# imjaegyun/super_resolution

Hardware: AMD Instinct MI355X
Metric: SR output megapixels/sec, HAT-S x4, 1280x720 LR in (higher is better)
Workload: dtype bf16; 1 GPU; HAT-S x4, one 3x720x1280 LR frame per GPU, full-frame forward; upscale=4, parallelism=dp1

## Files before the change

super_resolution_amd/build.py:

```python
from __future__ import annotations

import os
import subprocess
import sys
from concurrent.futures import ThreadPoolExecutor

HERE = os.path.dirname(os.path.abspath(__file__))
CSRC = os.path.join(HERE, "csrc")
LIB = os.path.join(HERE, "libhat_mi355x.so")
SOURCES = ["hat_conv.hip", "hat_conv64r.hip", "hat_attn.hip", "hat_misc.hip", "hat_ffn.hip", "hat_ffn2.hip", "hat_tail3.hip", "hat_tail3l.hip", "hat_pw.hip", "hat_mlp.hip", "hat_cabsq.hip", "hat_esc13.hip", "hat_plan.cpp"]
HEADERS = [os.path.join(CSRC, "hat_common.h"), os.path.join(os.path.dirname(HERE), "include", "hat_mi355x.h")]
FLAGS = ["-O3", "--offload-arch=gfx950", "-fPIC", "-std=c++17", "-Wall", "-Wno-unused-function"]


def _hipcc() -> str:
    for c in (os.environ.get("HIPCC"), "/opt/rocm/bin/hipcc", "hipcc"):
        if c and (os.path.isabs(c) and os.path.exists(c) or not os.path.isabs(c)):
            return c
    raise RuntimeError("hipcc not found")


def _stale(target: str, deps) -> bool:
    if not os.path.exists(target):
        return True
    t = os.path.getmtime(target)
    return any(os.path.getmtime(d) > t for d in deps)


def build(force: bool = False, verbose: bool = True) -> str:
    hipcc = _hipcc()
    objs, jobs = [], []
    for src in SOURCES:
        s = os.path.join(CSRC, src)
        o = os.path.join(CSRC, os.path.splitext(src)[0] + ".o")
        objs.append(o)
        if force or _stale(o, [s] + HEADERS):
            jobs.append([hipcc, *FLAGS, "-c", s, "-o", o])

    def run(cmd):
        if verbose:
            print(" ".join(cmd), flush=True)
        r = subprocess.run(cmd, capture_output=True, text=True)
        if r.returncode != 0:
            raise RuntimeError(f"hipcc failed:\n{' '.join(cmd)}\n{r.stdout}\n{r.stderr}")
        if verbose and r.stderr.strip():
            print(r.stderr, file=sys.stderr)

    with ThreadPoolExecutor(max_workers=4) as ex:
        list(ex.map(run, jobs))
    if force or jobs or _stale(LIB, objs):
        run([hipcc, "--offload-arch=gfx950", "-shared", "-fPIC", "-o", LIB, *objs])
    return LIB


if __name__ == "__main__":
    print(build(force="--force" in sys.argv))
```

super_resolution_amd/csrc/hat_tail3.hip:

```cpp
#include "hat_common.h"

#ifndef T3_ISSUE_ALL
#define T3_ISSUE_ALL 0
#endif
#ifndef T3_APF
#define T3_APF 1
#endif
#ifndef T3_S0RD
#define T3_S0RD 8
#endif
#ifndef T3_ABL
#define T3_ABL 0
#endif
#ifndef T3_USTORE_IL
#define T3_USTORE_IL 1
#endif
#ifndef T3_DMA_LATE
#define T3_DMA_LATE 0
#endif

namespace {

typedef _Float16 h2 __attribute__((ext_vector_type(2)));
typedef _Float16 h8 __attribute__((ext_vector_type(8)));
// ... 415 lines not shown
            };
            const bool pair16 = d.ldn % 8 == 0 && reinterpret_cast<uintptr_t>(d.n_out) % 16 == 0;
            {
                const f32x4 o0 = lnv(0);
                if (valid) {
                    if (4 * g < d.gap_c) gapv += as_stored<bf16_t>(o0);
                    if (d.n16_out != nullptr)
                        Vec4<bf16_t>::store(reinterpret_cast<bf16_t*>(d.n16_out) + ((size_t)b * H * W + pix) * 16 + 4 * g, o0);
                }
                if (pair16) {
                    store_pair_bf16_if(nout, 0, g, o0, lnv(1), valid);
#pragma unroll
                    for (int nt = 2; nt + 1 < NT; nt += 2) store_pair_bf16_if(nout, nt * 16, g, lnv(nt), lnv(nt + 1), valid);
                    if (valid) Vec4<bf16_t>::store(nout + (NT - 1) * 16 + 4 * g, lnv(NT - 1));
                } else if (valid) {
                    Vec4<bf16_t>::store(nout + 4 * g, o0);
#pragma unroll
                    for (int nt = 1; nt < NT; ++nt) Vec4<bf16_t>::store(nout + nt * 16 + 4 * g, lnv(nt));
                }
            }
        }
    }
    if constexpr (DBG & 64) {
        stamp(7);
        if (lane == 0) {
            const size_t wg = ((size_t)blockIdx.z * gridDim.y + blockIdx.y) * gridDim.x + blockIdx.x;
            for (int i = 0; i < 12; ++i) d.gap_out[(wg * T3_WAVES + wave) * 12 + i] = (float)tph[i];
        }
        return;
    }
    if (do_ln && d.gap_out != nullptr) {
        float* red = reinterpret_cast<float*>(smem + T3_WD_OFF);
#pragma unroll
        for (int r = 0; r < 4; ++r) {
            float s = gapv[r];
            s = row_sum16(s);
            if (c16 == 0) red[wave * 16 + 4 * g + r] = s;
        }
        __syncthreads();
        if (tid < 16) {
            float s = 0.f;
#pragma unroll
            for (int w = 0; w < T3_WAVES; ++w) s += red[w * 16 + tid];
            const size_t tile = (size_t)blockIdx.y * gridDim.x + blockIdx.x;
            d.gap_out[((size_t)b * gridDim.x * gridDim.y + tile) * 16 + tid] = tid < d.gap_c ? s : 0.f;
        }
    }
}

}

#ifndef HAT_TAIL3_NO_ENTRY
int hat_tail3_launch_c180(const HatHabTailDesc& h, void* stream);

extern "C" int hat_hab_tail3(const HatHabTailDesc* dp, void* stream) {
    if (!dp) return HAT_EINVAL;
    const HatHabTailDesc& h = *dp;
    const HatFfnDesc& d = h.ffn;
    if (!d.t_in || !d.t_out || d.t_in == d.t_out || !d.w1f || !d.dww || !d.w2f || !d.b2) return HAT_EINVAL;
    if (d.B < 1 || d.H < 1 || d.W < 1 || d.chunks < 1 || d.m_in) return HAT_EINVAL;
    if (d.dtype != HAT_BF16) return HAT_EUNSUPPORTED;
    if (d.C == 180) return (d.chunks == 12 && h.reserved1 == 0) ? hat_tail3_launch_c180(h, stream) : HAT_EINVAL;
    if (d.C != T3_C) return HAT_EUNSUPPORTED;
    if (d.ln1_g && (!d.ln1_b || !d.n_out || d.ldn < d.C || d.ldn % 4 || d.gap_c < 0 || d.gap_c > 16 || d.gap_c % 4)) return HAT_EINVAL;
    if (!h.n || !h.y16 || !h.c1 || !h.w_aggr || !h.wf || !h.bias_b || h.ldn_in < T3_C || h.ldn_in % 8) return HAT_EINVAL;
    const T3Aggr ag{reinterpret_cast<const bf16_t*>(h.n), reinterpret_cast<const bf16_t*>(h.y16), reinterpret_cast<const bf16_t*>(h.c1),
                    reinterpret_cast<const char*>(h.w_aggr), reinterpret_cast<const char*>(h.wf), h.bias_b, h.ldn_in};
    const int th = h.reserved1 & 3;
    if ((h.reserved1 & ~3) != 0) return HAT_EINVAL;
    if ((th & 1) && reinterpret_cast<uintptr_t>(d.t_in) % 8) return HAT_EINVAL;
    if ((th & 2) && reinterpret_cast<uintptr_t>(d.t_out) % 16) return HAT_EINVAL;
    void (*kern)(const HatFfnDesc, const T3Aggr) = th == 0 ? tail3_kernel<0, 0> : th == 1 ? tail3_kernel<0, 1> : th == 2 ? tail3_kernel<0, 2> : tail3_kernel<0, 3>;
    hipError_t e = hipFuncSetAttribute(reinterpret_cast<const void*>(kern), hipFuncAttributeMaxDynamicSharedMemorySize, T3_LDS);
    if (e != hipSuccess) return (int)e;
    dim3 grid((d.W + 15) / 16, (d.H + T3_ROWS - 1) / T3_ROWS, d.B);
    HAT_LAUNCH(kern, grid, dim3(256), T3_LDS, reinterpret_cast<hipStream_t>(stream), d, ag);
    return hat_check_launch();
}
#endif
```

super_resolution_amd/engine.py:

```python
from __future__ import annotations

import collections
import dataclasses
import math
import os
import threading
from typing import Dict, Optional

import torch

from . import ops
from .ops import (ACT_GELU, ACT_LRELU, ACT_NONE, O_NCHW_F32, O_NHWC_F32, O_NHWC_T, O_PIXSHUF_T, X_NCHW_F32_MEAN, X_NHWC_F32, X_NHWC_T)

RGB_MEAN = (0.4488, 0.4371, 0.4040)


def _r8(x: int) -> int:
    return (x + 7) // 8 * 8


def _r4(x: int) -> int:
    return (x + 3) // 4 * 4


@dataclasses.dataclass(frozen=True)
class Options:
    no_n16: bool = False
    no_t16: bool = False
    emu_t16: Optional[torch.dtype] = None
    no_fused_ffn: bool = False
    ffn_v1: bool = False
    no_hab_tail: bool = False
    tail_v2: bool = False
    no_cab_fold: bool = False
    no_cab_sweep: bool = False
    no_esc13: bool = False
    esc_side: bool = False
    one_stream: bool = False
    no_attn_log2: bool = False
    no_ocab_mlp: bool = False
    no_ocab_qkv: bool = False
    no_bf16_conv_in: bool = False
    no_conv_ln: bool = False

    @classmethod
    def from_env(cls, env=None) -> "Options":
        env = os.environ if env is None else env
        get = lambda name: env.get("HAT_" + name.upper(), "")
        any_value = ("no_cab_fold", "no_cab_sweep", "no_ocab_mlp", "no_ocab_qkv", "no_bf16_conv_in", "no_conv_ln")
        kw = {k.name: (get(k.name) != "" if k.name in any_value else get(k.name) == "1") for k in dataclasses.fields(cls)}
        return cls(**dict(kw, emu_t16={"fp16": torch.float16, "bf16": torch.bfloat16}.get(get("emu_t16"))))


class _ESC:

    def __init__(self, sd, core: str, plk_key: str, pdim: int, ksize: int, C: int, dtype: int, dev):
        f32 = dict(dtype=torch.float32, device=dev)
        self.pdim, self.ksize = pdim, ksize
        self.w1 = sd[core + ".plk.dwc_proj.1.weight"].detach().reshape(pdim // 2, pdim).to(**f32).contiguous()
        self.b1 = sd[core + ".plk.dwc_proj.1.bias"].detach().to(**f32).contiguous()
        self.w2 = sd[core + ".plk.dwc_proj.3.weight"].detach().reshape(pdim * 9, pdim // 2).to(**f32).contiguous()
        self.b2 = sd[core + ".plk.dwc_proj.3.bias"].detach().to(**f32).contiguous()
        lk = ops.pack_conv_weight(sd[plk_key], None, ops.HAT_F32, dev, nt=1)
        kc = ops.KC[dtype] * 3
        self.kpad = -(-(ksize * ksize * _r8(pdim)) // kc) * kc
        self.npad = 16 if pdim <= 16 else 32
        plk = torch.zeros(self.npad, self.kpad, **f32)
        plk[:lk.w.shape[0], :min(self.kpad, lk.kpad)] = lk.w[:self.npad, :min(self.kpad, lk.kpad)]
        self.plk = plk.contiguous()
        self.zero_bias = torch.zeros(self.npad, **f32)
        self.aggr = None
        self.aggr_keys = (core + ".aggr.weight", core + ".aggr.bias")
        self.conv13 = False


class _Packed:

    def __getitem__(self, key):
        try:
            return getattr(self, key)
        except AttributeError:
            raise KeyError(key) from None


class _Hab(_Packed):
    fold = ffn = ffn3 = fc1 = fc2 = bias256 = None
# ... 513 lines not shown
            self._esc_conv(esc, w, w["n"], B, H, W, n16=n16)
        s0.wait_stream(s1)

    def _fold_band(self, f: _Fwd, hb: _Hab, gst):
        w, bd, W, fo = f.w, f.band, f.W, hb.fold
        self._squeeze_chain(f, hb)
        st, c1, lo, own = w["cstat_l"], w["c1"], bd.lo, bd.own
        f.pooled(c1, 8, 8, st, 0)
        f.pooled(c1, 8, 8, st, 24, c0=0, c1=1)
        f.pooled(c1, 8, 8, st, 32, c0=W - 1, c1=W)
        if bd.r0 == 0:
            f.pooled(c1, 8, 8, st, 8, r0=lo, r1=lo + 1)
            f.pooled(c1, 8, 8, st, 40, r0=lo, r1=lo + 1, c0=0, c1=1)
            f.pooled(c1, 8, 8, st, 48, r0=lo, r1=lo + 1, c0=W - 1, c1=W)
        if bd.r1 == bd.Hfull:
            f.pooled(c1, 8, 8, st, 16, r0=lo + own - 1, r1=lo + own)
            f.pooled(c1, 8, 8, st, 56, r0=lo + own - 1, r1=lo + own, c0=0, c1=1)
            f.pooled(c1, 8, 8, st, 64, r0=lo + own - 1, r1=lo + own, c0=W - 1, c1=W)
        yield ("reduce", [(gst[0], gst[1], hb.esc.pdim), (st, w["cstat_g"], 72)])
        ops.cab_fold(None, None, 1, hb.cab0.npad, fo["w2"], fo["b2"], hb.eca_w, hb.eca_w.numel(), fo["ba"],
                     float(self.cfg["conv_scale"]), w["scale"], w["wf"], w["bias_b"], None, B=f.B, H=bd.Hfull, W=W, C_=self.C,
                     mid=hb.cab0.nout, dtype=f.dt, stats=w["cstat_g"], w2f=fo["w2f"])

    def _prologue_plain(self, f: _Fwd, hb: _Hab, gst):
        w, esc, bd, B, H, W, C, ldc = f.w, hb.esc, f.band, f.B, f.H, f.W, self.C, f.ldc
        mid = hb.cab0.nout
        c3 = ops.conv3x3_small if hb.cab0.frag else ops.conv
        c3(hb.cab0, w["n"], w["c1"], **f.geo, ldx=ldc, ldo=_r8(mid), act=ACT_GELU, n_store=_r4(mid))
        c3 = ops.conv3x3_small if hb.cab2.frag else ops.conv
        c3(hb.cab2, w["c1"], w["c2"], **f.geo, ldx=_r8(mid), ldo=ldc, colsum=w["colsum"])
        if bd is None:
            ops.eca_scale(w["colsum"], w["tiles"], hb.cab2.npad, f.N, hb.eca_w, hb.eca_w.numel(),
                          float(self.cfg["conv_scale"]), w["eca_tmp"], w["scale"], B=B, C_=C)
            self._esc_lk(esc, w, w["n"], B, H, W, f.nblk)
            return
        npd = hb.cab2.npad
        el, eg = (w[k].view(-1)[:B * npd].view(B, npd) for k in ("estat_l", "estat_g"))
        f.pooled(w["c2"], ldc, C, el)
        yield ("reduce", [(gst[0], gst[1], esc.pdim), (el, eg, _r4(C))])
        ops.eca_scale(eg, 1, npd, bd.Hfull * W, hb.eca_w, hb.eca_w.numel(), float(self.cfg["conv_scale"]), w["eca_tmp"],
                      w["scale"], B=B, C_=C)
        self._esc_w(esc, w, B, bd.Hfull, W, 1, gap=gst[1])
        self._esc_conv(esc, w, w["n"], B, H, W)

    def _tail_fused144(self, f: _Fwd, hb: _Hab):
        w, t = f.w, f.t
        if hb.out16:
            tout = w["hB"] if t is not w["hB"] else w["hC"]
        else:
            tout = w["tB"] if t is not w["tB"] else w["tC"]
        nxt, gap_c = hb.next_ln
        ops.hab_tail(hb.ffn3 if hb.ffn3 is not None else hb.ffn, hb.esc.aggr, t, tout, hb.n2[0], hb.n2[1], n=w["n"], ldn_in=f.ldc,
                     y16=w["y16"], c1=w["c1"], wf=w["wf"], bias_b=w["bias_b"], B=f.B, H=f.H, W=f.W, dtype=f.dt, ln1=nxt,
                     n_out=w["n2b"], ldn=f.ldc, gap_out=w["gap"], gap_c=gap_c, n16_out=(w["n16"] if self.use_n16 else None))
        w["n"], w["n2b"] = w["n2b"], w["n"]
        if self.opt.emu_t16 is not None:
            tout.copy_(tout.to(self.opt.emu_t16).to(torch.float32))
        f.t, f.have_n, f.have_n16, f.nblk = tout, True, self.use_n16, ops.ffn_tiles(hb.ffn, f.H, f.W, f.dt)

    def _tail_fused180(self, f: _Fwd, hb: _Hab):
        w, t = f.w, f.t
        tout = w["tB"] if t is not w["tB"] else w["tC"]
        nxt, gap_c = hb.next_ln
        ops.hab_tail(hb.ffn3, hb.esc.aggr, t, tout, hb.n2[0], hb.n2[1], n=w["n"], ldn_in=f.ldc, y16=w["y16"], bias_b=hb.bias256,
                     B=f.B, H=f.H, W=f.W, dtype=f.dt, ln1=nxt, n_out=w["n2b"], ldn=f.ldc, gap_out=w["gap"], gap_c=gap_c,
                     n16_out=(w["n16"] if self.use_n16 else None), r2=w["c2"], ldr2=f.ldc, r2scale=w["scale"],
                     r2scale_bstride=hb.cab2.npad)
        w["n"], w["n2b"] = w["n2b"], w["n"]
        f.t, f.have_n, f.have_n16, f.nblk = tout, True, self.use_n16, -(-f.H // 8) * -(-f.W // 16)

    def _tail_aggr_cab(self, f: _Fwd, hb: _Hab):
        w = f.w
        ops.aggr_cab(hb.esc.aggr, w["n"], w["tB"], w["c1"], w["wf"], w["bias_b"], **f.geo, ldx=f.ldc, ldo=self.C, x0=w["y16"],
                     c_split=hb.esc.pdim, ldx0=w["y16"].shape[2], r1=f.t, ldr1=self.C)
        self._ffn(f, hb)

    def _tail_aggr(self, f: _Fwd, hb: _Hab):
        w = f.w
        self._run_lin(hb.esc.aggr, w["n"], w["tB"], **f.geo, ldx=f.ldc, ldo=self.C, out_mode=O_NHWC_F32, x0=w["y16"],
                      c_split=hb.esc.pdim, ldx0=w["y16"].shape[2], r1=f.t, ldr1=self.C, r2=w["c2"], ldr2=f.ldc,
                      r2scale=w["scale"], r2scale_bstride=hb.cab2.npad)
        self._ffn(f, hb)

    def _ffn(self, f: _Fwd, hb: _Hab):
        w, C, ldc = f.w, self.C, f.ldc
        tB, tC = w["tB"], w["tC"]
        if hb.ffn is not None:
            nxt, gap_c = hb.next_ln
            if gap_c > 16:
                ops.ffn(hb.ffn, tB, tC, hb.n2[0], hb.n2[1], B=f.B, H=f.H, W=f.W, dtype=f.dt)
                f.t, f.have_n, f.have_n16 = tC, False, False
            else:
                ops.ffn(hb.ffn, tB, tC, hb.n2[0], hb.n2[1], B=f.B, H=f.H, W=f.W, dtype=f.dt, ln1=nxt, n_out=w["n"], ldn=ldc,
                        gap_out=w["gap"], gap_c=gap_c)
                f.t, f.have_n, f.have_n16, f.nblk = tC, True, False, ops.ffn_tiles(hb.ffn, f.H, f.W, f.dt)
            return
        f.ln(tB, w["n"], hb.n2)
        hid2 = hb.fc1.nout
        self._run_lin(hb.fc1, w["n"], w["u"], **f.geo, ldx=ldc, ldo=w["u"].shape[2])
        if self.hatx:
            ops.sgfn_gate(w["u"], hb.dw_w, hb.dw_b, w["g"], B=f.B, H=f.H, W=f.W, half=hid2 // 2, ldu=w["u"].shape[2],
                          ldo=w["g"].shape[2], dtype=f.dt)
        else:
            ops.dwconv_gate(w["u"], hb.dw_w, hb.dw_b, w["g"], B=f.B, H=f.H, W=f.W, hid=hid2 // 2, ldu=w["u"].shape[2],
                            ldo=w["g"].shape[2], dtype=f.dt)
        self._run_lin(hb.fc2, w["g"], tB, **f.geo, ldx=w["g"].shape[2], ldo=C, out_mode=O_NHWC_F32, r1=tB, ldr1=C)
        f.t, f.have_n, f.have_n16 = tB, False, False
# ... 126 lines not shown
```

super_resolution_amd/ops.py:

```python
from __future__ import annotations

import ctypes as C
from typing import Optional

import torch

from . import _lib
from ._lib import (ACT_GELU, ACT_LRELU, ACT_NONE, HAT_BF16, HAT_F32, O_NCHW_F32, O_NHWC_F32, O_NHWC_T, O_PIXSHUF_T,
                   X_NCHW_F32_MEAN, X_NHWC_F32, X_NHWC_T, HatAggrCabDesc, HatCabFoldDesc, HatConvDesc, HatFfnDesc, HatHabTailDesc, HatMlpDesc)

TORCH_DTYPE = {HAT_F32: torch.float32, HAT_BF16: torch.bfloat16}
DTYPE_CODE = {"f32": HAT_F32, "fp32": HAT_F32, "float32": HAT_F32, "bf16": HAT_BF16, "bfloat16": HAT_BF16}
KC = {HAT_F32: 32, HAT_BF16: 64}


def _ptr(t: Optional[torch.Tensor]) -> Optional[int]:
    if t is None:
        return None
    if not t.is_cuda:
        raise RuntimeError("HAT HIP ops need device tensors (no CPU path exists)")
    if not t.is_contiguous():
        raise RuntimeError("HAT HIP ops need contiguous tensors")
    return t.data_ptr()

# ... 563 lines not shown
    d = HatFfnDesc()
    d.B, d.H, d.W, d.C, d.chunks, d.dtype = B, H, W, pf.C, pf.chunks, dtype
    return d


def ffn_tiles(pf: PackedFFN, H: int, W: int, dtype: int) -> int:
    lib = _lib.load()
    d = _ffn_desc(pf, 1, H, W, dtype)
    n = C.c_int32(0)
    _lib.check(lib.hat_ffn_tiles(C.byref(d), C.byref(n)), "hat_ffn_tiles")
    return n.value


def ffn_m_ld(C_: int) -> int:
    return (C_ + 1 + 31) // 32 * 32


def _fill_ffn(d, pf: PackedFFN, t_in, t_out, ln_g, ln_b, ln1, n_out, ldn, gap_out, gap_c, m_in=None, ldm_in=0, n16_out=None):
    d.t_in, d.t_out, d.ln_g, d.ln_b = _ptr(t_in), _ptr(t_out), _ptr(ln_g), _ptr(ln_b)
    if m_in is not None:
        d.m_in, d.ldm_in = _ptr(m_in), ldm_in
    d.w1f, d.b1, d.dww, d.dwb, d.w2f, d.b2 = _ptr(pf.w1f), _ptr(pf.b1), _ptr(pf.dww), _ptr(pf.dwb), _ptr(pf.w2f), _ptr(pf.b2)
    if ln1 is not None:
        d.ln1_g, d.ln1_b, d.n_out, d.ldn = _ptr(ln1[0]), _ptr(ln1[1]), _ptr(n_out), ldn
        d.gap_out, d.gap_c = (_ptr(gap_out) if gap_c else None), gap_c
        d.n16_out = _ptr(n16_out)


def ffn(pf: PackedFFN, t_in, t_out, ln_g, ln_b, *, B: int, H: int, W: int, dtype: int, ln1=None, n_out=None, ldn: int = 0,
        gap_out=None, gap_c: int = 0, m_in=None, ldm_in: int = 0):
    lib = _lib.load()
    d = _ffn_desc(pf, B, H, W, dtype)
    _fill_ffn(d, pf, t_in, t_out, ln_g, ln_b, ln1, n_out, ldn, gap_out, gap_c, m_in, ldm_in)
    flops = B * H * W * (2.0 * pf.C * 2 * pf.hid + 2.0 * 9 * 2 * pf.hid + 2.0 * pf.hid * pf.C)
    es = 2 if dtype == HAT_BF16 else 4
    nbytes = B * H * W * (4.0 * pf.C + 4.0 * pf.C + (es * ldn if ln1 is not None else 0) + (es * ldm_in if m_in is not None else 0))
    if pf.khalf == "v3":
        raise RuntimeError("a hat_hab_tail3-packed FFN has no stand-alone launch: pack with pack_ffn2 for hat_ffn2")
    if pf.khalf == "v2":
        _timed("ffn2_kernel", flops, lambda: _lib.check(lib.hat_ffn2(C.byref(d), _stream()), "hat_ffn2"), nbytes=nbytes)
        return
    _timed(f"ffn_kernel<{_TNAME[dtype]}>", flops, lambda: _lib.check(lib.hat_ffn(C.byref(d), _stream()), "hat_ffn"),
           nbytes=nbytes)


def hab_tail_supported(pf: PackedFFN, aggr: PackedConv, mid: int, dtype: int) -> bool:
    if pf.C == 180:
        return pf.khalf == "v3" and aggr.frag and aggr.nt == 12 and aggr.n_slices == 1 and aggr.kpad == 192 and dtype == HAT_BF16
    return pf.khalf in ("v2", "v3") and aggr.frag and aggr.nt == 9 and aggr.n_slices == 1 and aggr.kpad == 160 and mid <= 8 and dtype == HAT_BF16


def hab_tail(pf: PackedFFN, aggr: PackedConv, t_in, t_out, ln_g, ln_b, *, n, ldn_in: int, y16, c1=None, wf=None, bias_b, B: int, H: int,
             W: int, dtype: int, ln1=None, n_out=None, ldn: int = 0, gap_out=None, gap_c: int = 0, n16_out=None,
             r2=None, ldr2: int = 0, r2scale=None, r2scale_bstride: int = 0):
    lib = _lib.load()
    h = HatHabTailDesc()
    d = h.ffn
    d.B, d.H, d.W, d.C, d.chunks, d.dtype = B, H, W, pf.C, pf.chunks, dtype
    _fill_ffn(d, pf, t_in, t_out, ln_g, ln_b, ln1, n_out, ldn, gap_out, gap_c, n16_out=n16_out)
    h.n, h.y16, h.c1, h.w_aggr, h.wf, h.bias_b, h.ldn_in = _ptr(n), _ptr(y16), _ptr(c1), _ptr(aggr.w), _ptr(wf), _ptr(bias_b), ldn_in
    h.r2, h.ldr2, h.r2scale, h.r2scale_bstride = _ptr(r2), ldr2, _ptr(r2scale), r2scale_bstride
    in_half, out_half = t_in.dtype == torch.float16, t_out.dtype == torch.float16
    if (in_half or out_half) and not (pf.C == 144 and pf.khalf == "v3"):
        raise RuntimeError("an FP16 residual stream is only instantiated for hat_hab_tail3 at embed_dim 144")
    if (not in_half and t_in.dtype != torch.float32) or (not out_half and t_out.dtype != torch.float32):
        raise RuntimeError("hab_tail: t_in / t_out must be fp32 or FP16 rows")
    h.reserved1 = (1 if in_half else 0) | (2 if out_half else 0)
    if pf.C == 180:
        flops = B * H * W * (2.0 * pf.C * pf.C + 2.0 * pf.C * 2 * pf.hid + 2.0 * 9 * 2 * pf.hid + 2.0 * pf.hid * pf.C)
        nbytes = B * H * W * (2.0 * ldn_in + 32 + 2.0 * ldr2 + 4.0 * pf.C + 4.0 * pf.C + (2 * ldn if ln1 is not None else 0))
        _timed("tail3l_kernel", flops, lambda: _lib.check(lib.hat_hab_tail3(C.byref(h), _stream()), "hat_hab_tail3"), nbytes=nbytes)
        return
    flops = B * H * W * (2.0 * pf.C * (pf.C + 72) + 2.0 * pf.C * 2 * pf.hid + 2.0 * 9 * 2 * pf.hid + 2.0 * pf.hid * pf.C)
    nbytes = B * H * W * (2.0 * ldn_in + 32 + 16 + (2.0 if in_half else 4.0) * pf.C + (2.0 if out_half else 4.0) * pf.C + (2 * ldn if ln1 is not None else 0))
    if pf.khalf == "v3":
        _timed("tail3_kernel", flops, lambda: _lib.check(lib.hat_hab_tail3(C.byref(h), _stream()), "hat_hab_tail3"), nbytes=nbytes)
        return
    _timed("ffn2_kernel<aggr>", flops, lambda: _lib.check(lib.hat_hab_tail(C.byref(h), _stream()), "hat_hab_tail"), nbytes=nbytes)


_PW_SHAPES = {(9, 5), (18, 5), (9, 9), (12, 6), (23, 6), (12, 12), (4, 1), (4, 2)}


def choose_nt_linear(nout: int, cin: int, dtype: int):
    if nout == 288 and -(-cin // 32) == 5 and dtype == HAT_BF16:
        return 18, 1
    if nout == 360 and -(-cin // 32) == 6 and dtype == HAT_BF16:
        return 23, 1
    return choose_nt(nout)


def linear_supported(nout: int, cin: int, dtype: int) -> bool:
    nt, _ = choose_nt_linear(nout, cin, dtype)
    ks = -(-cin // 32)
    lds = nt * ks * 64 * 8 * (2 if dtype == HAT_BF16 else 4)
    return (nt, ks) in _PW_SHAPES and lds <= 163840 and cin % 4 == 0


def pack_linear_weight(weight: torch.Tensor, bias: Optional[torch.Tensor], dtype: int, device, scale: float = 1.0) -> PackedConv:
    w = weight.detach().to(torch.float32).cpu()
    ksize, cin = 1, None
    if w.dim() == 4 and w.shape[-1] > 1:
        o_, i_, ksize, _ = w.shape
        cin, cin_p = i_, (i_ + 7) // 8 * 8
        wt = torch.zeros(o_, ksize * ksize, cin_p)
        wt[:, :, :i_] = w.permute(0, 2, 3, 1).reshape(o_, ksize * ksize, i_)
        w = wt.reshape(o_, -1)
    w = w.reshape(w.shape[0], -1) * scale
    o, i = w.shape
    b = (torch.zeros(o) if bias is None else bias.detach().to(torch.float32).cpu()) * scale
    nt, n_slices = choose_nt_linear(o, i, dtype) if ksize == 1 else choose_nt(o)
    ks = -(-i // 32)
    npad = nt * 16 * n_slices
    wp = torch.zeros(npad, ks * 32)
    wp[:o, :i] = w
    lane = torch.arange(64)
    row = (torch.arange(n_slices)[:, None, None, None, None] * nt * 16 + torch.arange(nt)[None, :, None, None, None] * 16
           + (lane & 15)[None, None, None, :, None]).expand(n_slices, nt, ks, 64, 8)
    col = (torch.arange(ks)[None, None, :, None, None] * 32 + 8 * (lane >> 4)[None, None, None, :, None]
           + torch.arange(8)[None, None, None, None, :]).expand(n_slices, nt, ks, 64, 8)
# ... 112 lines not shown
```

Before: 345.7 MP/s.

## Add 8-wave tail3 kernel pairing two row tiles with staggered FFN phases

Adds a new 512-thread tail3p kernel in which two 4-wave halves each process a row tile and share double-buffered W1/W2/depthwise weight DMA per chunk. The halves run the pointwise and depthwise/W2 phases one step apart, so one half's MFMA work overlaps the other's LDS work, and each weight chunk is loaded once for both tiles. It becomes the default for the C=144 hat_hab_tail3 path, and the old 4-wave kernel stays reachable through a tail3_4w option. The kernel uses a larger LDS footprint at one workgroup per CU and carries added synchronisation complexity.

```diff
diff --git a/super_resolution_amd/build.py b/super_resolution_amd/build.py
--- a/super_resolution_amd/build.py
+++ b/super_resolution_amd/build.py
@@ -8,7 +8,7 @@
 HERE = os.path.dirname(os.path.abspath(__file__))
 CSRC = os.path.join(HERE, "csrc")
 LIB = os.path.join(HERE, "libhat_mi355x.so")
-SOURCES = ["hat_conv.hip", "hat_conv64r.hip", "hat_attn.hip", "hat_misc.hip", "hat_ffn.hip", "hat_ffn2.hip", "hat_tail3.hip", "hat_tail3l.hip", "hat_pw.hip", "hat_mlp.hip", "hat_cabsq.hip", "hat_esc13.hip", "hat_plan.cpp"]
+SOURCES = ["hat_conv.hip", "hat_conv64r.hip", "hat_attn.hip", "hat_misc.hip", "hat_ffn.hip", "hat_ffn2.hip", "hat_tail3.hip", "hat_tail3p.hip", "hat_tail3l.hip", "hat_pw.hip", "hat_mlp.hip", "hat_cabsq.hip", "hat_esc13.hip", "hat_plan.cpp"]
 HEADERS = [os.path.join(CSRC, "hat_common.h"), os.path.join(os.path.dirname(HERE), "include", "hat_mi355x.h")]
 FLAGS = ["-O3", "--offload-arch=gfx950", "-fPIC", "-std=c++17", "-Wall", "-Wno-unused-function"]
 
diff --git a/super_resolution_amd/csrc/hat_tail3.hip b/super_resolution_amd/csrc/hat_tail3.hip
--- a/super_resolution_amd/csrc/hat_tail3.hip
+++ b/super_resolution_amd/csrc/hat_tail3.hip
@@ -491,6 +491,7 @@
 
 #ifndef HAT_TAIL3_NO_ENTRY
 int hat_tail3_launch_c180(const HatHabTailDesc& h, void* stream);
+int hat_tail3p_launch_c144(const HatHabTailDesc& h, int th, void* stream);
 
 extern "C" int hat_hab_tail3(const HatHabTailDesc* dp, void* stream) {
     if (!dp) return HAT_EINVAL;
@@ -506,9 +507,10 @@
     const T3Aggr ag{reinterpret_cast<const bf16_t*>(h.n), reinterpret_cast<const bf16_t*>(h.y16), reinterpret_cast<const bf16_t*>(h.c1),
                     reinterpret_cast<const char*>(h.w_aggr), reinterpret_cast<const char*>(h.wf), h.bias_b, h.ldn_in};
     const int th = h.reserved1 & 3;
-    if ((h.reserved1 & ~3) != 0) return HAT_EINVAL;
+    if ((h.reserved1 & ~7) != 0) return HAT_EINVAL;
     if ((th & 1) && reinterpret_cast<uintptr_t>(d.t_in) % 8) return HAT_EINVAL;
     if ((th & 2) && reinterpret_cast<uintptr_t>(d.t_out) % 16) return HAT_EINVAL;
+    if (!(h.reserved1 & 4)) return hat_tail3p_launch_c144(h, th, stream);
     void (*kern)(const HatFfnDesc, const T3Aggr) = th == 0 ? tail3_kernel<0, 0> : th == 1 ? tail3_kernel<0, 1> : th == 2 ? tail3_kernel<0, 2> : tail3_kernel<0, 3>;
     hipError_t e = hipFuncSetAttribute(reinterpret_cast<const void*>(kern), hipFuncAttributeMaxDynamicSharedMemorySize, T3_LDS);
     if (e != hipSuccess) return (int)e;
diff --git a/super_resolution_amd/csrc/hat_tail3p.hip b/super_resolution_amd/csrc/hat_tail3p.hip
--- /dev/null
+++ b/super_resolution_amd/csrc/hat_tail3p.hip
@@ -0,0 +1,470 @@
+#ifndef HAT_TAIL3_NO_ENTRY
+#define HAT_TAIL3P_ENTRY
+#define HAT_TAIL3_NO_ENTRY
+#endif
+#include "hat_tail3.hip"
+
+#ifndef T3P_PRIO
+#define T3P_PRIO 0
+#endif
+
+namespace {
+
+constexpr int T3P_WAVES = 8;
+constexpr int T3P_US_BYTES = T3_NPH * T3_US_ROWB;
+constexpr int T3P_W1_OFF = 2 * T3P_US_BYTES;
+constexpr int T3P_W2_BYTES = T3_NT * 1024;
+constexpr int T3P_W2_OFF = T3P_W1_OFF + 2 * T3_W1_BYTES;
+constexpr int T3P_WD_OFF = T3P_W2_OFF + 2 * T3P_W2_BYTES;
+constexpr int T3P_LDS = T3P_WD_OFF + 2 * T3_WD_REC;
+static_assert(T3_B2_OFF + 1024 <= T3P_LDS && T3P_LDS <= 160 * 1024, "LDS map");
+static_assert(T3_B2_OFF + 1024 <= T3P_W2_OFF, "stage 0 must not overlap the W2 / Wd buffers");
+
+template <int DBG, int TH = 0>
+__global__ __launch_bounds__(512, 1) void tail3p_kernel(const HatFfnDesc d, const T3Aggr ag) {
+    constexpr int C = T3_C, NT = T3_NT, KS = T3_KS, HALO_W = T3_HW;
+    extern __shared__ __attribute__((aligned(16))) char smem[];
+    const unsigned lds0 = (unsigned)(uintptr_t)(lds_char*)smem;
+
+    const int tid = threadIdx.x, lane = tid & 63, g = lane >> 4, c16 = lane & 15;
+    const int wv = __builtin_amdgcn_readfirstlane(tid >> 6);
+    const int half = wv >> 2, wave = wv & 3;
+    if constexpr (T3P_PRIO != 0) {
+        if (half) __builtin_amdgcn_s_setprio(1);
+    }
+    const int b = blockIdx.z, x0 = blockIdx.x * 16, y0 = blockIdx.y * (2 * T3_ROWS) + half * T3_ROWS;
+    const int H = d.H, W = d.W;
+    const float* tin = d.t_in + (size_t)b * H * W * C;
+    const _Float16* tinh = reinterpret_cast<const _Float16*>(d.t_in) + (size_t)b * H * W * C;
+    const unsigned usb = lds0 + (unsigned)(half * T3P_US_BYTES);
+
+    long long tph[12] = {0, 0, 0, 0, 0, 0, 0, 0, 0, 0, 0, 0};
+    long long tlast = 0;
+    auto stamp = [&](int slot) {
+        if constexpr (DBG & 64) {
+            const long long now = (long long)__builtin_amdgcn_s_memtime();
+            tph[slot] += now - tlast;
+            tlast = now;
+        }
+    };
+    if constexpr (DBG & 64) tlast = (long long)__builtin_amdgcn_s_memtime();
+
+    const char* w1g = reinterpret_cast<const char*>(d.w1f);
+    const char* w2g = reinterpret_cast<const char*>(d.w2f);
+    const char* wdg = reinterpret_cast<const char*>(d.dww);
+    const unsigned lane16 = (unsigned)lane * 16u;
+    auto dma_chunk = [&](int c, int c1, int buf1) {
+#pragma unroll
+        for (int j = 0; j < 4; ++j) {
+            const int f = 8 * j + wv;
+            const int fr = f - 20, fd = f == 30 ? 1024 : 0;
+            const char* src = f < 20 ? w1g + ((size_t)c1 * T3_W1_BYTES + f * 1024)
+                            : fr < 9 ? w2g + ((size_t)c * T3P_W2_BYTES + fr * 1024) : wdg + ((size_t)c * T3_WD_REC + fd);
+            char* dst = f < 20 ? smem + T3P_W1_OFF + buf1 * T3_W1_BYTES + f * 1024
+                      : fr < 9 ? smem + T3P_W2_OFF + (c & 1) * T3P_W2_BYTES + fr * 1024 : smem + T3P_WD_OFF + (c & 1) * T3_WD_REC + fd;
+            dma1k(src, lane16, dst);
+        }
+    };
+
+    f32x4 acc2[NT][2];
+    bf8 mb[3][KS];
+    int hp[3];
+    {
+        {
+            const char* wfb = ag.wf + (size_t)b * NT * 3 * 1024;
+#pragma unroll
+            for (int j = 0; j < 10; ++j) {
+                const int f = wv * 10 + j, nt = f >> 3, ks = f & 7;
+                const char* src = f >= 72 ? reinterpret_cast<const char*>(d.b2)
+                                : ks < 5 ? ag.wl + (size_t)(nt * 5 + ks) * 1024 : wfb + (size_t)(nt * 3 + ks - 5) * 1024;
+                dma1k(src, lane16, smem + (f >= 72 ? T3_B2_OFF : f * 1024));
+            }
+        }
+        __builtin_amdgcn_sched_barrier(0);
+        bool ins[3];
+        bf8 bfr[3][8];
+        f32x4 accx[NT];
+        typedef unsigned u32x2h __attribute__((ext_vector_type(2)));
+        u32x2h thr[3][TH & 1 ? NT : 1];
+        const bf16_t* nb = ag.n + (size_t)b * H * W * ag.ldn;
+        const bf16_t* yb = ag.y16 + (size_t)b * H * W * 16;
+        const bf16_t* cb = ag.c1 + (size_t)b * H * W * 8;
+        auto issue_tile = [&](int t) {
+            int hy, hx;
+            if (t < 2) { hy = 2 * wave + 1 + t; hx = 1 + c16; }
+            else if (wave < 2) { hy = wave * (T3_ROWS + 1); hx = 1 + c16; }
+            else { const int jj = wave == 2 ? c16 : (c16 & 3); hy = (wave == 2 ? 0 : 8) + (jj >> 1); hx = (jj & 1) * (HALO_W - 1); }
+            const int y = y0 - 1 + hy, x = x0 - 1 + hx;
+            ins[t] = y >= 0 && y < H && x >= 0 && x < W;
+            const int yc = min(max(y, 0), H - 1), xc = min(max(x, 0), W - 1);
+            hp[t] = hy * HALO_W + hx;
+            const int pix = yc * W + xc;
+#pragma unroll
+            for (int ks = 0; ks < 5; ++ks) {
+                const int c = ks * 32 + 8 * g;
+                const bf16_t* src = c < 16 ? yb + (size_t)pix * 16 + c : nb + (size_t)pix * ag.ldn + min(c, C - 8);
+                bfr[t][ks] = MT<bf16_t>::load(src);
+            }
+#pragma unroll
+            for (int kc = 0; kc < 3; ++kc) {
+                const int tap = 4 * kc + g;
+                const int dy = tap / 3 - 1, dx = tap - (tap / 3) * 3 - 1;
+                const int yy = yc + dy, xx = xc + dx;
+                const bool inb = tap < 9 && yy >= 0 && yy < H && xx >= 0 && xx < W;
+                const bf16_t* cst = reinterpret_cast<const bf16_t*>(tap == 9 ? hat_tail3_ones_page : hat_tail3_zero_page);
+                bfr[t][5 + kc] = MT<bf16_t>::load(inb ? cb + ((size_t)yy * W + xx) * 8 : cst);
+            }
+#pragma unroll
+            for (int nt = 0; nt < NT; ++nt) {
+                if constexpr (TH & 1) {
+                    thr[t][nt] = *reinterpret_cast<const u32x2h*>(tinh + (size_t)pix * C + nt * 16 + 4 * g);
+                } else {
+                    const f32x4 tv = *reinterpret_cast<const f32x4*>(tin + (size_t)pix * C + nt * 16 + 4 * g);
+                    if (t < 2) acc2[nt][t] = tv; else accx[nt] = tv;
+                }
+            }
+            __builtin_amdgcn_sched_barrier(0);
+        };
+        issue_tile(2);
+        issue_tile(0);
+        if constexpr (T3_ISSUE_ALL) issue_tile(1);
+        stamp(8);
+        if constexpr (T3_ISSUE_ALL) asm volatile("s_waitcnt vmcnt(51)" ::: "memory");
+        else asm volatile("s_waitcnt vmcnt(34)" ::: "memory");
+        lds_barrier();
+        stamp(9);
+        typedef unsigned u32x2 __attribute__((ext_vector_type(2)));
+#pragma unroll
+        for (int o = 0; o < 3; ++o) {
+            const int t = o == 0 ? 2 : o - 1;
+            f32x4 v[NT];
+#pragma unroll
+            for (int nt = 0; nt < NT; ++nt) {
+                if constexpr (TH & 1) {
+                    const h2 lo = as_h2(thr[t][nt][0]), hi = as_h2(thr[t][nt][1]);
+                    v[nt] = f32x4{(float)lo[0], (float)lo[1], (float)hi[0], (float)hi[1]};
+                } else {
+                    v[nt] = t == 2 ? accx[nt] : acc2[nt][t];
+                }
+            }
+            constexpr int RD = T3_S0RD;
+            u32x4 ar[RD];
+#pragma unroll
+            for (int i = 0; i < RD; ++i) ar[i] = lds_rd16(lds0 + (unsigned)(i * 1024) + lane16);
+#pragma unroll
+            for (int i = 0; i < NT * 8; ++i) {
+                const int nt = i >> 3, ks = i & 7;
+                v[nt] = __builtin_amdgcn_mfma_f32_16x16x32_bf16(__builtin_bit_cast(bf8, ar[i % RD]), bfr[t][ks], v[nt], 0, 0, 0);
+                if (i + RD < NT * 8) ar[i % RD] = lds_rd16(lds0 + (unsigned)((i + RD) * 1024) + lane16);
+                __builtin_amdgcn_sched_barrier(0);
+            }
+            __builtin_amdgcn_sched_barrier(0);
+            if (o == 0 && !T3_ISSUE_ALL) issue_tile(1);
+            float s = 0.f;
+#pragma unroll
+            for (int nt = 0; nt < NT; ++nt) s += (v[nt][0] + v[nt][1]) + (v[nt][2] + v[nt][3]);
+            s += __shfl_xor(s, 16); s += __shfl_xor(s, 32);
+            const float mean = s * (1.0f / (float)C);
+            float q = 0.f;
+#pragma unroll
+            for (int nt = 0; nt < NT; ++nt)
+#pragma unroll
+                for (int r = 0; r < 4; ++r) { const float dl = v[nt][r] - mean; q += dl * dl; }
+            q += __shfl_xor(q, 16); q += __shfl_xor(q, 32);
+            const float rstd = ins[t] ? __builtin_amdgcn_rsqf(q * (1.0f / (float)C) + 1e-5f) : 0.f;
+            const float nmr = -mean * rstd;
+            typedef bf16_t v4b __attribute__((ext_vector_type(4)));
+            u32x2 pk[NT + 1];
+#pragma unroll
+            for (int nt = 0; nt < NT; ++nt) {
+                const v4b hb = {(bf16_t)(v[nt][0] * rstd + nmr), (bf16_t)(v[nt][1] * rstd + nmr), (bf16_t)(v[nt][2] * rstd + nmr),
+                                (bf16_t)(v[nt][3] * rstd + nmr)};
+                pk[nt] = __builtin_bit_cast(u32x2, hb);
+                if (t < 2) acc2[nt][t] = v[nt] + __builtin_bit_cast(f32x4, lds_rd16(lds0 + T3_B2_OFF + (unsigned)(nt * 64 + g * 16)));
+            }
+            pk[NT] = u32x2{(g == 0 && ins[t]) ? 0x00003F80u : 0u, 0u};
+#pragma unroll
+            for (int ks = 0; ks < KS; ++ks) {
+                const auto r0 = __builtin_amdgcn_permlane32_swap(pk[2 * ks][0], pk[2 * ks + 1][0], false, false);
+                const auto r1 = __builtin_amdgcn_permlane32_swap(pk[2 * ks][1], pk[2 * ks + 1][1], false, false);
+                const auto s0 = __builtin_amdgcn_permlane16_swap(r0[0], r0[1], false, false);
+                const auto s1 = __builtin_amdgcn_permlane16_swap(r1[0], r1[1], false, false);
+                mb[t][ks] = __builtin_bit_cast(bf8, u32x4{s0[0], s1[0], s0[1], s1[1]});
+            }
+            __builtin_amdgcn_sched_barrier(0);
+        }
+        stamp(10);
+        lds_barrier();
+        stamp(11);
+#pragma unroll
+        for (int j = 0; j < 3; ++j) {
+            const int f = 8 * j + wv, fp = f < 20 ? f : f - 20;
+            dma1k(w1g + fp * 1024, lane16, smem + T3P_W1_OFF + fp * 1024);
+        }
+    }
+
+    unsigned ust[3];
+#pragma unroll
+    for (int t = 0; t < 3; ++t) ust[t] = usb + (unsigned)(hp[t] * T3_US_ROWB + g * 16);
+    const unsigned ubase = usb + (unsigned)((2 * wave * HALO_W + c16) * T3_US_ROWB + g * 16);
+    const unsigned wdad0 = lds0 + T3P_WD_OFF + (unsigned)g * 320u;
+    const unsigned w2ad0 = lds0 + T3P_W2_OFF + lane16;
+
+    stamp(0);
+    asm volatile("s_waitcnt vmcnt(0)" ::: "memory");
+    lds_barrier();
+    stamp(1);
+
+    const int nc = d.chunks;
+    for (int k = 0; k <= 2 * nc; ++k) {
+        if (!(k & 1) && k < 2 * nc) {
+            const int c = k >> 1;
+            dma_chunk(c, min(c + 1, nc - 1), (c + 1) & 1);
+        }
+        const int j = k - half;
+        const bool busy = j >= 0 && j < 2 * nc;
+        const int chunk = j >> 1;
+        if (busy && !(j & 1)) {
+            const unsigned w1b = lds0 + T3P_W1_OFF + (unsigned)((chunk & 1) * T3_W1_BYTES) + lane16;
+            f32x4 acc[2][2][3] = {};
+            auto store_u1 = [&](int p, int t) {
+                u32x4 pk;
+#pragma unroll
+                for (int ii = 0; ii < 2; ++ii) {
+                    pk[2 * ii] = __builtin_bit_cast(unsigned, __builtin_amdgcn_cvt_pkrtz(acc[p][ii][t][0], acc[p][ii][t][1]));
+                    pk[2 * ii + 1] = __builtin_bit_cast(unsigned, __builtin_amdgcn_cvt_pkrtz(acc[p][ii][t][2], acc[p][ii][t][3]));
+                }
+                *(__attribute__((address_space(3))) u32x4*)(uintptr_t)(ust[t] + (unsigned)(p * 64)) = pk;
+            };
+            auto store_u = [&](int p) {
+#pragma unroll
+                for (int t = 0; t < 3; ++t) store_u1(p, t);
+            };
+            constexpr int APF = T3_APF, NSTEP = 2 * KS;
+            u32x4 ar[APF + 1][2];
+            auto rd_a = [&](int step) {
+                const int p1 = step / KS, k1 = step % KS;
+                ar[step % (APF + 1)][0] = lds_rd16(w1b + (unsigned)(((2 * p1) * KS + k1) * 1024));
+                ar[step % (APF + 1)][1] = lds_rd16(w1b + (unsigned)(((2 * p1 + 1) * KS + k1) * 1024));
+            };
+#pragma unroll
+            for (int i = 0; i < APF; ++i) rd_a(i);
+#pragma unroll
+            for (int p = 0; p < 2; ++p) {
+#pragma unroll
+                for (int ks = 0; ks < KS; ++ks) {
+                    const int step = p * KS + ks;
+                    if (step + APF < NSTEP) rd_a(step + APF);
+#pragma unroll
+                    for (int ii = 0; ii < 2; ++ii) {
+#pragma unroll
+                        for (int t = 0; t < 3; ++t) {
+                            const f32x4 c0 = ks == 0 ? f32x4{0.f, 0.f, 0.f, 0.f} : acc[p][ii][t];
+                            acc[p][ii][t] = __builtin_amdgcn_mfma_f32_16x16x32_bf16(__builtin_bit_cast(bf8, ar[step % (APF + 1)][ii]), mb[t][ks], c0, 0, 0, 0);
+                        }
+                        if (T3_USTORE_IL && p == 1 && ii == 0 && ks >= 1 && ks <= 3) store_u1(0, ks - 1);
+                    }
+                    __builtin_amdgcn_sched_barrier(0);
+                }
+                if (!T3_USTORE_IL && p == 1) store_u(0);
+            }
+            store_u(1);
+            stamp(2);
+        } else if (busy) {
+            unsigned wdad = wdad0 + (unsigned)((chunk & 1) * T3_WD_REC), w2ad = w2ad0 + (unsigned)((chunk & 1) * T3P_W2_BYTES);
+            asm volatile("" : "+v"(wdad), "+v"(w2ad));
+            h2 da[2][4], dg[2][4];
+            {
+                const u32x4 ba = lds_rd16(wdad + 9 * 32), bg = lds_rd16(wdad + 9 * 32 + 16);
+#pragma unroll
+                for (int pt = 0; pt < 2; ++pt)
+#pragma unroll
+                    for (int k4 = 0; k4 < 4; ++k4) { da[pt][k4] = as_h2(ba[k4]); dg[pt][k4] = as_h2(bg[k4]); }
+            }
+            {
+                constexpr int PD = 3;
+                u32x4 wa[2][3], wg[2][3], ua[PD + 1], ug[PD + 1];
+                auto rd_w = [&](int tr, int dx) {
+                    wa[tr & 1][dx] = lds_rd16(wdad + (unsigned)((tr * 3 + dx) * 32));
+                    wg[tr & 1][dx] = lds_rd16(wdad + (unsigned)((tr * 3 + dx) * 32 + 16));
+                };
+                auto rd_u = [&](int pos) {
+                    const int hr = pos / 3, dx = pos - 3 * hr;
+                    ua[pos % (PD + 1)] = lds_rd16(ubase + (unsigned)((hr * HALO_W + dx) * T3_US_ROWB));
+                    ug[pos % (PD + 1)] = lds_rd16(ubase + (unsigned)((hr * HALO_W + dx) * T3_US_ROWB + 64));
+                };
+#pragma unroll
+                for (int dx = 0; dx < 3; ++dx) rd_w(0, dx);
+#pragma unroll
+                for (int p = 0; p < PD; ++p) rd_u(p);
+#pragma unroll
+                for (int dx = 0; dx < 3; ++dx) rd_w(1, dx);
+#pragma unroll
+                for (int pos = 0; pos < 12; ++pos) {
+                    const int hr = pos / 3, dx = pos - 3 * hr;
+                    if (pos + PD < 12) rd_u(pos + PD);
+                    __builtin_amdgcn_sched_barrier(0);
+                    const u32x4 cua = ua[pos % (PD + 1)], cug = ug[pos % (PD + 1)];
+                    if (hr < 3) {
+#pragma unroll
+                        for (int k4 = 0; k4 < 4; ++k4) {
+                            da[0][k4] = as_h2(wa[hr & 1][dx][k4]) * as_h2(cua[k4]) + da[0][k4];
+                            dg[0][k4] = as_h2(wg[hr & 1][dx][k4]) * as_h2(cug[k4]) + dg[0][k4];
+                        }
+                    }
+                    if (hr >= 1) {
+#pragma unroll
+                        for (int k4 = 0; k4 < 4; ++k4) {
+                            da[1][k4] = as_h2(wa[(hr - 1) & 1][dx][k4]) * as_h2(cua[k4]) + da[1][k4];
+                            dg[1][k4] = as_h2(wg[(hr - 1) & 1][dx][k4]) * as_h2(cug[k4]) + dg[1][k4];
+                        }
+                    }
+                    __builtin_amdgcn_sched_barrier(0);
+                    if (hr >= 1 && hr + 1 < 3) rd_w(hr + 1, dx);
+                }
+            }
+            stamp(4);
+            h8 a2[NT];
+#pragma unroll
+            for (int nt = 0; nt < NT; ++nt) a2[nt] = __builtin_bit_cast(h8, lds_rd16(w2ad + (unsigned)(nt * 1024)));
+#pragma unroll
+            for (int pt = 0; pt < 2; ++pt) {
+                u32x4 gu;
+#pragma unroll
+                for (int k4 = 0; k4 < 4; ++k4) {
+                    const h2 x = dg[pt][k4];
+                    const h2 tt = x * (h2){(_Float16)-1.4426950408889634f, (_Float16)-1.4426950408889634f};
+                    h2 e = {(_Float16)__builtin_exp2f16(tt[0]), (_Float16)__builtin_exp2f16(tt[1])};
+                    e = e + (h2){(_Float16)1.0f, (_Float16)1.0f};
+                    const h2 r = {(_Float16)__builtin_amdgcn_rcph(e[0]), (_Float16)__builtin_amdgcn_rcph(e[1])};
+                    gu[k4] = as_u(da[pt][k4] * (x * r));
+                }
+                const h8 gf = __builtin_bit_cast(h8, gu);
+#pragma unroll
+                for (int nt = 0; nt < NT; ++nt) acc2[nt][pt] = __builtin_amdgcn_mfma_f32_16x16x32_f16(a2[nt], gf, acc2[nt][pt], 0, 0, 0);
+            }
+            stamp(5);
+        }
+        if (!(k & 1)) asm volatile("s_waitcnt vmcnt(0)" ::: "memory");
+        lds_barrier();
+        if (!busy) stamp(1);
+        else if (j & 1) stamp(6);
+        else stamp(3);
+    }
+
+    float* tout = d.t_out + (size_t)b * H * W * C;
+    const bool do_ln = d.ln1_g != nullptr;
+    f32x4 gapv = {0.f, 0.f, 0.f, 0.f};
+    f32x4 g1v[NT], bt1v[NT];
+    if (do_ln) {
+#pragma unroll
+        for (int nt = 0; nt < NT; ++nt) {
+            g1v[nt] = *reinterpret_cast<const f32x4*>(d.ln1_g + nt * 16 + 4 * g);
+            bt1v[nt] = *reinterpret_cast<const f32x4*>(d.ln1_b + nt * 16 + 4 * g);
+        }
+    }
+#pragma unroll
+    for (int pt = 0; pt < 2; ++pt) {
+        const int y = y0 + 2 * wave + pt, x = x0 + c16;
+        const bool valid = y < H && x < W;
+        const size_t pix = (size_t)y * W + x;
+        float s = 0.f;
+#pragma unroll
+        for (int nt = 0; nt < NT; ++nt) {
+            const f32x4 v = acc2[nt][pt];
+            if constexpr (!(TH & 2)) { if (valid) *reinterpret_cast<f32x4*>(tout + pix * C + nt * 16 + 4 * g) = v; }
+            s += (v[0] + v[1]) + (v[2] + v[3]);
+        }
+        if constexpr ((TH & 2) != 0) {
+            _Float16* trow = reinterpret_cast<_Float16*>(d.t_out) + ((size_t)b * H * W + pix) * C;
+#pragma unroll
+            for (int nt = 0; nt + 1 < NT; nt += 2) store_pair_f16_if(trow, nt * 16, g, acc2[nt][pt], acc2[nt + 1][pt], valid);
+            if (valid) {
+                typedef _Float16 v4h __attribute__((ext_vector_type(4)));
+                const f32x4 v = acc2[NT - 1][pt];
+                auto c = [](float x) { return (_Float16)__builtin_amdgcn_fmed3f(x, -65504.0f, 65504.0f); };
+                *reinterpret_cast<v4h*>(trow + (NT - 1) * 16 + 4 * g) = v4h{c(v[0]), c(v[1]), c(v[2]), c(v[3])};
+            }
+        }
+        if (do_ln) {
+            s += __shfl_xor(s, 16); s += __shfl_xor(s, 32);
+            const float mean = s / (float)C;
+            float q = 0.f;
+#pragma unroll
+            for (int nt = 0; nt < NT; ++nt)
+#pragma unroll
+                for (int r = 0; r < 4; ++r) { const float dl = acc2[nt][pt][r] - mean; q += dl * dl; }
+            q += __shfl_xor(q, 16); q += __shfl_xor(q, 32);
+            const float rstd = 1.0f / sqrtf(q / (float)C + 1e-5f);
+            bf16_t* nout = reinterpret_cast<bf16_t*>(d.n_out) + ((size_t)b * H * W + pix) * d.ldn;
+            auto lnv = [&](int nt) {
+                f32x4 o;
+#pragma unroll
+                for (int r = 0; r < 4; ++r) o[r] = (acc2[nt][pt][r] - mean) * rstd * g1v[nt][r] + bt1v[nt][r];
+                return o;
+            };
+            const bool pair16 = d.ldn % 8 == 0 && reinterpret_cast<uintptr_t>(d.n_out) % 16 == 0;
+            {
+                const f32x4 o0 = lnv(0);
+                if (valid) {
+                    if (4 * g < d.gap_c) gapv += as_stored<bf16_t>(o0);
+                    if (d.n16_out != nullptr)
+                        Vec4<bf16_t>::store(reinterpret_cast<bf16_t*>(d.n16_out) + ((size_t)b * H * W + pix) * 16 + 4 * g, o0);
+                }
+                if (pair16) {
+                    store_pair_bf16_if(nout, 0, g, o0, lnv(1), valid);
+#pragma unroll
+                    for (int nt = 2; nt + 1 < NT; nt += 2) store_pair_bf16_if(nout, nt * 16, g, lnv(nt), lnv(nt + 1), valid);
+                    if (valid) Vec4<bf16_t>::store(nout + (NT - 1) * 16 + 4 * g, lnv(NT - 1));
+                } else if (valid) {
+                    Vec4<bf16_t>::store(nout + 4 * g, o0);
+#pragma unroll
+                    for (int nt = 1; nt < NT; ++nt) Vec4<bf16_t>::store(nout + nt * 16 + 4 * g, lnv(nt));
+                }
+            }
+        }
+    }
+    if constexpr (DBG & 64) {
+        stamp(7);
+        if (lane == 0) {
+            const size_t wg = ((size_t)blockIdx.z * gridDim.y + blockIdx.y) * gridDim.x + blockIdx.x;
+            for (int i = 0; i < 12; ++i) d.gap_out[(wg * T3P_WAVES + wv) * 12 + i] = (float)tph[i];
+        }
+        return;
+    }
+    if (do_ln && d.gap_out != nullptr) {
+        float* red = reinterpret_cast<float*>(smem + T3P_WD_OFF);
+#pragma unroll
+        for (int r = 0; r < 4; ++r) {
+            float s = gapv[r];
+            s = row_sum16(s);
+            if (c16 == 0) red[wv * 16 + 4 * g + r] = s;
+        }
+        __syncthreads();
+        const int hh = tid >> 4, ch = tid & 15, ty = blockIdx.y * 2 + hh;
+        if (tid < 32 && ty * T3_ROWS < H) {
+            float s = 0.f;
+#pragma unroll
+            for (int w = 0; w < 4; ++w) s += red[(hh * 4 + w) * 16 + ch];
+            const size_t nty = (size_t)(H + T3_ROWS - 1) / T3_ROWS;
+            const size_t tile = (size_t)ty * gridDim.x + blockIdx.x;
+            d.gap_out[((size_t)b * gridDim.x * nty + tile) * 16 + ch] = ch < d.gap_c ? s : 0.f;
+        }
+    }
+}
+
+}
+
+#ifdef HAT_TAIL3P_ENTRY
+int hat_tail3p_launch_c144(const HatHabTailDesc& h, int th, void* stream) {
+    const HatFfnDesc& d = h.ffn;
+    const T3Aggr ag{reinterpret_cast<const bf16_t*>(h.n), reinterpret_cast<const bf16_t*>(h.y16), reinterpret_cast<const bf16_t*>(h.c1),
+                    reinterpret_cast<const char*>(h.w_aggr), reinterpret_cast<const char*>(h.wf), h.bias_b, h.ldn_in};
+    void (*kern)(const HatFfnDesc, const T3Aggr) = th == 0 ? tail3p_kernel<0, 0> : th == 1 ? tail3p_kernel<0, 1> : th == 2 ? tail3p_kernel<0, 2> : tail3p_kernel<0, 3>;
+    hipError_t e = hipFuncSetAttribute(reinterpret_cast<const void*>(kern), hipFuncAttributeMaxDynamicSharedMemorySize, T3P_LDS);
+    if (e != hipSuccess) return (int)e;
+    dim3 grid((d.W + 15) / 16, (d.H + 2 * T3_ROWS - 1) / (2 * T3_ROWS), d.B);
+    HAT_LAUNCH(kern, grid, dim3(512), T3P_LDS, reinterpret_cast<hipStream_t>(stream), d, ag);
+    return hat_check_launch();
+}
+#endif
diff --git a/super_resolution_amd/engine.py b/super_resolution_amd/engine.py
--- a/super_resolution_amd/engine.py
+++ b/super_resolution_amd/engine.py
@@ -32,6 +32,7 @@
     ffn_v1: bool = False
     no_hab_tail: bool = False
     tail_v2: bool = False
+    tail3_4w: bool = False
     no_cab_fold: bool = False
     no_cab_sweep: bool = False
     no_esc13: bool = False
@@ -651,7 +652,8 @@
         nxt, gap_c = hb.next_ln
         ops.hab_tail(hb.ffn3 if hb.ffn3 is not None else hb.ffn, hb.esc.aggr, t, tout, hb.n2[0], hb.n2[1], n=w["n"], ldn_in=f.ldc,
                      y16=w["y16"], c1=w["c1"], wf=w["wf"], bias_b=w["bias_b"], B=f.B, H=f.H, W=f.W, dtype=f.dt, ln1=nxt,
-                     n_out=w["n2b"], ldn=f.ldc, gap_out=w["gap"], gap_c=gap_c, n16_out=(w["n16"] if self.use_n16 else None))
+                     n_out=w["n2b"], ldn=f.ldc, gap_out=w["gap"], gap_c=gap_c, n16_out=(w["n16"] if self.use_n16 else None),
+                     tail3_4w=self.opt.tail3_4w and hb.ffn3 is not None)
         w["n"], w["n2b"] = w["n2b"], w["n"]
         if self.opt.emu_t16 is not None:
             tout.copy_(tout.to(self.opt.emu_t16).to(torch.float32))
diff --git a/super_resolution_amd/ops.py b/super_resolution_amd/ops.py
--- a/super_resolution_amd/ops.py
+++ b/super_resolution_amd/ops.py
@@ -639,7 +639,7 @@
 
 def hab_tail(pf: PackedFFN, aggr: PackedConv, t_in, t_out, ln_g, ln_b, *, n, ldn_in: int, y16, c1=None, wf=None, bias_b, B: int, H: int,
              W: int, dtype: int, ln1=None, n_out=None, ldn: int = 0, gap_out=None, gap_c: int = 0, n16_out=None,
-             r2=None, ldr2: int = 0, r2scale=None, r2scale_bstride: int = 0):
+             r2=None, ldr2: int = 0, r2scale=None, r2scale_bstride: int = 0, tail3_4w: bool = False):
     lib = _lib.load()
     h = HatHabTailDesc()
     d = h.ffn
@@ -652,7 +652,9 @@
         raise RuntimeError("an FP16 residual stream is only instantiated for hat_hab_tail3 at embed_dim 144")
     if (not in_half and t_in.dtype != torch.float32) or (not out_half and t_out.dtype != torch.float32):
         raise RuntimeError("hab_tail: t_in / t_out must be fp32 or FP16 rows")
-    h.reserved1 = (1 if in_half else 0) | (2 if out_half else 0)
+    if tail3_4w and not (pf.C == 144 and pf.khalf == "v3"):
+        raise RuntimeError("tail3_4w selects between hat_hab_tail3's two kernels at embed_dim 144")
+    h.reserved1 = (1 if in_half else 0) | (2 if out_half else 0) | (4 if tail3_4w else 0)
     if pf.C == 180:
         flops = B * H * W * (2.0 * pf.C * pf.C + 2.0 * pf.C * 2 * pf.hid + 2.0 * 9 * 2 * pf.hid + 2.0 * pf.hid * pf.C)
         nbytes = B * H * W * (2.0 * ldn_in + 32 + 2.0 * ldr2 + 4.0 * pf.C + 4.0 * pf.C + (2 * ldn if ln1 is not None else 0))
```

Measured after the change: 294.7 MP/s, median of 2. 0.852x the previous value.
